# nyu-systems/Grendel-GS

Measured on AMD Instinct MI355X. Metric: training iters/sec (fwd+bwd), higher is better.
Workload: dtype f32

## Files before the change

grendel-gs_amd/csrc/api.hip:

```cpp
#include "common.h"

extern "C" {

const char *gsr_error_string(int code) {
    if (code == 0) return "success";
    if (code == GSR_EINVAL) return "gsraster: invalid argument";
    if (code == GSR_ENOSPACE) return "gsraster: workspace too small";
    if (code == GSR_ERETRY) return "gsraster: pair count valid, bounded sort must be repeated";
    if (code == GSR_EFAULT)
        return "gsraster: a persistent binning kernel of an earlier call timed out at a grid barrier (hung or preempted "
               "device); that view's lists are incomplete; the look-back pipeline is used from now on";
    if (code > 0) return hipGetErrorString((hipError_t)code);
    return "gsraster: unknown error";
}

int gsr_abi_version(void) { return 14; }

int gsr_get_block_xy(int *block_x, int *block_y, int *one_dim_block) {
    if (!block_x || !block_y || !one_dim_block) return GSR_EINVAL;
    *block_x = GSR_BLOCK_X;
    *block_y = GSR_BLOCK_Y;
    *one_dim_block = GSR_ONE_DIM_BLOCK;
    return 0;
}
// ... 189 lines not shown
                              const uint8_t *compute_locally, const float *bg, const float *final_T,
                              const int32_t *n_contrib, const float *dL_dpixels, float *dL_record,
                              const float *out_color, void *seg_ws, size_t seg_bytes, int row_lo, int row_hi,
                              int record_is_zero, double *acc64, uint8_t *touched, gsr_stream_t stream) {
    if (P < 0 || width <= 0 || height <= 0) return GSR_EINVAL;
    if (P == 0) return 0;
    if (!ranges || !compute_locally || !bg || !final_T || !n_contrib || !dL_dpixels || !means2D || !conic_opacity ||
        !rgb || !dL_record || !acc64)
        return GSR_EINVAL;
    return gsr_launch_composite_backward(P, width, height, ranges, point_list, means2D, conic_opacity, rgb,
                                         compute_locally, bg, final_T, n_contrib, dL_dpixels, dL_record, out_color,
                                         seg_ws, seg_bytes, row_lo, row_hi, record_is_zero ? 1 : 0,
                                         reinterpret_cast<hipStream_t>(stream), acc64, touched);
}

int gsr_render_backward(int P, int width, int height, const int32_t *ranges, const uint32_t *point_list,
                        const float *means2D, const float *conic_opacity, const float *rgb,
                        const uint8_t *compute_locally, const float *bg, const float *final_T,
                        const int32_t *n_contrib, const float *dL_dpixels, float *dL_record, gsr_stream_t stream) {
    if (P < 0 || width <= 0 || height <= 0) return GSR_EINVAL;
    if (P == 0) return 0;
    if (!ranges || !compute_locally || !bg || !final_T || !n_contrib || !dL_dpixels || !means2D || !conic_opacity ||
        !rgb || !dL_record)
        return GSR_EINVAL;
    return gsr_launch_composite_backward(P, width, height, ranges, point_list, means2D, conic_opacity, rgb,
                                         compute_locally, bg, final_T, n_contrib, dL_dpixels, dL_record, nullptr,
                                         nullptr, 0, 0, 0, 0, reinterpret_cast<hipStream_t>(stream));
}

}
// ... 1 lines not shown
```

grendel-gs_amd/csrc/common.h:

```cpp
#pragma once
#include <hip/hip_runtime.h>
#include <stdint.h>

#include "../../include/gsraster.h"

#define GSR_WAVE 64

#define GSR_LAUNCH_CHECK()                         \
    do {                                           \
        hipError_t e__ = hipGetLastError();        \
        if (e__ != hipSuccess) return (int)e__;    \
    } while (0)

#define GSR_HIP(expr)                              \
    do {                                           \
        hipError_t e__ = (expr);                   \
        if (e__ != hipSuccess) return (int)e__;    \
    } while (0)

static inline int gsr_div_up(long long a, long long b) { return (int)((a + b - 1) / b); }

__device__ __forceinline__ int gsr_xcd_span_of_block(int b, int nwg) {
#ifdef GSR_NO_XCD_MAP
    return b;
// ... 75 lines not shown
                                  hipStream_t stream);
int gsr_launch_preprocess_backward(int P, int D, int M, const float *means3D, const float *scales,
                                   float scale_modifier, const float *rotations, const float *shs,
                                   const float *shs_rest, const float *opacities_raw, const float *viewmatrix, const float *projmatrix, const float *campos, int W,
                                   int H, float tanfovx, float tanfovy, const int32_t *radii, const float *cov3D,
                                   const uint8_t *clamped, const float *dL_dmeans2D, const float *dL_dconic_opacity,
                                   const float *dL_drgb, int grad_row_stride, float *dL_dmeans3D, float *dL_dscales, float *dL_drotations,
                                   float *dL_dshs, float *dL_dshs_rest, float *dL_dopacities, hipStream_t stream);
int gsr_launch_local2j(int P, int W, int H, int ws, const float *means2D, const int32_t *radii, const int32_t *div,
                       uint8_t *out, hipStream_t stream);

int gsr_launch_composite_forward(int P, int W, int H, const int32_t *ranges, const uint32_t *point_list,
                                 const float *means2D, const float *conic_opacity, const float *rgb,
                                 const uint8_t *compute_locally, const float *bg, float *out_color, float *final_T,
                                 int32_t *n_contrib, void *seg_ws, size_t seg_bytes, int row_lo, int row_hi,
                                 void *zero_ptr, size_t zero_bytes, hipStream_t stream);
size_t gsr_composite_seg_bytes(int W, int H);
int gsr_launch_composite_backward(int P, int W, int H, const int32_t *ranges, const uint32_t *point_list,
                                  const float *means2D, const float *conic_opacity, const float *rgb,
                                  const uint8_t *compute_locally, const float *bg, const float *final_T,
                                  const int32_t *n_contrib, const float *dL_dpixels, float *dL_record,
                                  const float *out_color, void *seg_ws, size_t seg_bytes, int row_lo, int row_hi,
                                  int record_is_zero, hipStream_t stream, double *acc64 = nullptr,
                                  uint8_t *touched = nullptr);
```

grendel-gs_amd/csrc/composite.hip:

```cpp
#include "common.h"

namespace {

constexpr float LOG2E = 1.4426950408889634f;
constexpr float ALPHA_MIN = 1.0f / 255.0f;
constexpr float T_STOP = 0.0001f;

__device__ unsigned long long g_walked[2];

#ifdef GSR_STATS
__device__ unsigned long long g_stats[8];
#define GSR_STAT(i, v) do { const unsigned long long sv__ = (unsigned long long)(v); if (lane == 0) atomicAdd(&g_stats[i], sv__); } while (0)
#else
#define GSR_STAT(i, v) do { } while (0)
#endif

struct Entry {
    float x, y;
    float a2, b2, c2;
    float o;
    bool relevant;
};

#ifndef GSR_NO_LOG2O
// ... 125 lines not shown
    return 64 + sizeof(uint32_t) * (size_t)cap + sizeof(int32_t) * (size_t)tiles * SEG_MAXJ + sizeof(float) * 1024 * (size_t)cap;
}
inline SegWs seg_ws_of(void *ws, int tiles, uint32_t cap) {
    SegWs w{};
    if (!ws) return w;
    char *b = reinterpret_cast<char *>(ws);
    w.hdr = reinterpret_cast<uint32_t *>(b);
    w.queue = reinterpret_cast<uint32_t *>(b + 64);
    w.seg_slot = reinterpret_cast<int32_t *>(b + 64 + sizeof(uint32_t) * (size_t)cap);
    w.ckpt = reinterpret_cast<float *>(b + 64 + sizeof(uint32_t) * (size_t)cap + sizeof(int32_t) * (size_t)tiles * SEG_MAXJ);
    w.cap = cap;
    return w;
}
constexpr uint32_t SEG_CAP = 8192;

__device__ __forceinline__ void k8_checkpoint(const SegWs &seg, int *s_slot, int tile, int c, int lane,
                                                        int wave, float T, float c0, float c1, float c2) {
    const int j = c / SEG_LEN - 1;
    int slot = 0;
    if (lane == 0) {
        int v = atomicCAS(&s_slot[j], -1, -2);
        if (v == -1) {
            const uint32_t k = atomicAdd(seg.hdr, 1u);
            v = k < seg.cap ? (int)k : -3;
            if (v >= 0) {
                seg.queue[k] = (uint32_t)tile * 32u + (uint32_t)(j + 1);
                seg.seg_slot[(size_t)tile * SEG_MAXJ + j] = v;
            }
            __hip_atomic_store(&s_slot[j], v, __ATOMIC_RELEASE, __HIP_MEMORY_SCOPE_WORKGROUP);
        } else {
// ... 7 lines not shown
        ck[0] = T;
        ck[256] = c0;
        ck[512] = c1;
        ck[768] = c2;
    }
}

template <bool SEG, bool BAND>
__global__ void __launch_bounds__(256)
composite_forward_kernel(int W, int H, int gx, const int2 *__restrict__ ranges,
                         const uint32_t *__restrict__ point_list, const float2 *__restrict__ means2D,
                         const float4 *__restrict__ conic_opacity, const float *__restrict__ rgb,
                         const uint8_t *__restrict__ compute_locally, const float *__restrict__ bg,
                         float *__restrict__ out_color, float *__restrict__ final_T, int32_t *__restrict__ n_contrib,
                         const SegWs seg, int band_first, int band_tiles, uint4 *__restrict__ zero16,
                         size_t zero16_n) {
    const size_t HW = (size_t)H * W;
    for (size_t i = (size_t)blockIdx.x * 256 + threadIdx.x; i < zero16_n; i += (size_t)gridDim.x * 256)
        zero16[i] = make_uint4(0u, 0u, 0u, 0u);
    int tile;
    bool idle = false;
    if (BAND) {
        if (band_first < 0) {
            const int gy = (H + GSR_BLOCK_Y - 1) / GSR_BLOCK_Y;
            int2 hull = ranges[gx * gy];
            if (hull.x < 0 || hull.y > gy || hull.x >= hull.y) hull = make_int2(0, 0);
            band_first = hull.x * gx;
            band_tiles = min((hull.y - hull.x) * gx, band_tiles);
            idle = (int)blockIdx.x >= band_tiles;
        }
        tile = band_first + (idle ? 0 : gsr_xcd_span_of_block(blockIdx.x, band_tiles));
// ... 6 lines not shown
        const size_t p1 = (size_t)min(H, ((band_first + band_tiles) / gx) * GSR_BLOCK_Y) * W;
        const size_t nout = n0 + (HW - p1);
        for (size_t i = (size_t)blockIdx.x * 256 + threadIdx.x; i < nout; i += (size_t)gridDim.x * 256) {
            const size_t q = i < n0 ? i : p1 + (i - n0);
            out_color[q] = 0.f;
            out_color[HW + q] = 0.f;
            out_color[2 * HW + q] = 0.f;
            final_T[q] = 1.f;
            n_contrib[q] = 0;
        }
    };
    if (idle) {
        clear_outside();
        return;
    }
    const int lane = threadIdx.x & 63, wave = threadIdx.x >> 6;
    const int tx = tile % gx, ty = tile / gx;
    const int qx0 = tx * GSR_BLOCK_X + (wave & 1) * 8, qy0 = ty * GSR_BLOCK_Y + (wave >> 1) * 8;
    const int px = qx0 + (lane & 7), py = qy0 + (lane >> 3);
    const bool inside = px < W && py < H;
    const size_t pid = (size_t)py * W + px;

    if (!compute_locally[tile]) {
        if (inside) {
            out_color[pid] = 0.f;
            out_color[HW + pid] = 0.f;
            out_color[2 * HW + pid] = 0.f;
            final_T[pid] = 1.f;
            n_contrib[pid] = 0;
        }
        clear_outside();
// ... 30 lines not shown
        float r = 0.f, g = 0.f, b = 0.f;
        if (e.relevant) {
            r = rgb[3 * (size_t)id];
            g = rgb[3 * (size_t)id + 1];
            b = rgb[3 * (size_t)id + 2];
        }
        unsigned long long m = __ballot(e.relevant);
        GSR_STAT(0, __popcll(__ballot(have)));
        GSR_STAT(1, __popcll(m));
        const int nrel = __popcll(m);
        if (e.relevant) pair_store(wslab, __popcll(m & ((1ull << lane) - 1ull)), e, r, g, b);
        {
            const int pad = (-nrel) & 3, slot = nrel + lane / 9;
            if (lane < 9 * pad) wslab[(slot >> 1) * PREC + 2 * (lane % 9) + (slot & 1)] = 0.f;
        }
        for (int p0 = 0; p0 < nrel; p0 += 4) {
            float al[4];
            bool ok[4];
            int kk[4];
            v2f cr[2], cg[2], cb[2];
#pragma unroll
            for (int h = 0; h < 2; h++) {
                const PairRec pr = pair_load(wslab, (p0 >> 1) + h);
                const v2f pe = pair_exponent(pr, pxf, pyf);
                cr[h] = pr.r;
                cg[h] = pr.g;
                cb[h] = pr.b;
#pragma unroll
                for (int u = 0; u < 2; u++) {
                    const bool live = m != 0;
// ... 37 lines not shown
    if (inside) {
        out_color[pid] = C0 + T * bg[0];
        out_color[HW + pid] = C1 + T * bg[1];
        out_color[2 * HW + pid] = C2 + T * bg[2];
        final_T[pid] = T;
        n_contrib[pid] = last;
    }
    clear_outside();
}

typedef float f32x4 __attribute__((ext_vector_type(4)));

constexpr int MB = 8;
constexpr int MSTR = 66;

template <typename Acc>
__device__ __forceinline__ void
composite_backward_segment(const int tile, const int sidx, int W, int H, int gx, const int2 *__restrict__ ranges,
                           const uint32_t *__restrict__ point_list, const float2 *__restrict__ means2D,
                           const float4 *__restrict__ conic_opacity, const float *__restrict__ rgb,
                           const uint8_t *__restrict__ compute_locally, const float *__restrict__ bg,
                           const float *__restrict__ final_T, const int32_t *__restrict__ n_contrib,
                           const float *__restrict__ dL_dpixels, Acc *__restrict__ dL_record,
                           const float *__restrict__ out_color, const SegWs &seg, uint8_t *__restrict__ touched) {
    if (!compute_locally[tile]) return;
    const int lane = threadIdx.x & 63, wave = threadIdx.x >> 6;
    const int tx = tile % gx, ty = tile / gx;
    const int qx0 = tx * GSR_BLOCK_X + (wave & 1) * 8, qy0 = ty * GSR_BLOCK_Y + (wave >> 1) * 8;
    const int px = qx0 + (lane & 7), py = qy0 + (lane >> 3);
    const bool inside = px < W && py < H;
    const size_t pid = (size_t)py * W + px;
    const size_t HW = (size_t)H * W;
    const int2 range = ranges[tile];
    const float pxf = (float)px, pyf = (float)py;

    const int c_lo = sidx * SEG_LEN;
    int end_slot = -1;
    if (seg.seg_slot && sidx < SEG_MAXJ) end_slot = seg.seg_slot[(size_t)tile * SEG_MAXJ + sidx];
    const int c_hi = end_slot >= 0 ? c_lo + SEG_LEN : 0x7fffffff;
// ... 66 lines not shown

    float T = T_final;
    float rho = 0.f;
    if (end_slot >= 0 && last > c_hi) {
        const float *ck = seg.ckpt + (size_t)end_slot * 1024 + wave * 64 + lane;
        T = ck[0];
        const float r0 = out_color[pid] - T_final * bg[0] - ck[256];
        const float r1 = out_color[HW + pid] - T_final * bg[1] - ck[512];
        const float r2 = out_color[2 * HW + pid] - T_final * bg[2] - ck[768];
        rho = (r0 * g0 + r1 * g1 + r2 * g2) * __builtin_amdgcn_rcpf(T);
    }

    const int c0 = ((bmax - 1) / 64) * 64;
    uint32_t id_cur = (c0 + lane < wmax) ? point_list[range.x + c0 + lane] : 0u;
    uint32_t id_nxt = (c0 >= c_lo + 64 && c0 - 64 + lane < wmax) ? point_list[range.x + c0 - 64 + lane] : 0u;
    RawEntry raw = load_raw(c0 + lane < wmax, id_cur, means2D, conic_opacity, rgb);

    for (int c = c0; c >= c_lo; c -= 64) {
        float *acc_tab = sacc[wave];
        const bool have_nxt = c >= c_lo + 64 && c - 64 + lane < wmax;
        const RawEntry raw_nxt = load_raw(have_nxt, id_nxt, means2D, conic_opacity, rgb);
        const uint32_t id_nxt2 = (c >= c_lo + 128 && c - 128 + lane < wmax) ? point_list[range.x + c - 128 + lane] : 0u;
        if (c < wmax) {
            const bool have = c + lane < wmax;
            Entry e;
            e.x = raw.xy.x;
            e.y = raw.xy.y;
            e.a2 = -0.5f * LOG2E * raw.co.x;
            e.b2 = -LOG2E * raw.co.y;
            e.c2 = -0.5f * LOG2E * raw.co.z;
            e.o = entry_opacity_term(raw.co.w);
            e.relevant = have && gsr_can_touch_box(raw.xy, raw.co, (float)qx0, (float)qy0, (float)qx0 + 7.0f, (float)qy0 + 7.0f);
            unsigned long long m = __ballot(e.relevant);
            GSR_STAT(0, __popcll(__ballot(have)));
            GSR_STAT(1, __popcll(m));
            GSR_STAT(6, 1);
            if (e.relevant) pair_store(wslab, __popcll((m >> lane) >> 1), e, raw.r, raw.g, raw.b);
            if (wave == wbest) {
                float *fe = &fslab[7 * lane];
                fe[0] = e.x;  fe[1] = e.y;  fe[2] = e.a2;  fe[3] = e.b2;  fe[4] = e.c2;
                fe[5] = __uint_as_float(id_cur);
                fe[6] = raw.co.w;
            }
            unsigned long long sk = 0ull;
            auto contract_batch = [&](int filled) {
                __builtin_amdgcn_wave_barrier();
                f32x4 acc = {0.f, 0.f, 0.f, 0.f}, acc1 = {0.f, 0.f, 0.f, 0.f};
#pragma unroll
// ... 101 lines not shown
                if (val != 0.f) {
                    const uint32_t id = __float_as_uint(sout[10 * e + 9]);
                    atomicAdd(dL_record + 9 * (size_t)id + col, (Acc)val);
                    if (touched) touched[id] = 1;
                }
#else
                asm volatile("" ::"v"(val));
#endif
            }
        }
#pragma unroll
        for (int i = 0; i < 9; i++) acc_tab[64 * i + lane] = 0.f;
        raw = raw_nxt;
        id_cur = id_nxt;
        id_nxt = id_nxt2;
    }
}

template <typename Acc>
__global__ void __launch_bounds__(256, 4)
composite_backward_kernel(int W, int H, int gx, int tiles, const int2 *__restrict__ ranges,
                          const uint32_t *__restrict__ point_list, const float2 *__restrict__ means2D,
                          const float4 *__restrict__ conic_opacity, const float *__restrict__ rgb,
                          const uint8_t *__restrict__ compute_locally, const float *__restrict__ bg,
                          const float *__restrict__ final_T, const int32_t *__restrict__ n_contrib,
                          const float *__restrict__ dL_dpixels, Acc *__restrict__ dL_record,
                          const float *__restrict__ out_color, const SegWs seg, int band_first, int band_tiles,
                          uint8_t *__restrict__ touched) {
    const int nstatic = band_tiles > 0 ? band_tiles : tiles;
    const bool worker = (int)blockIdx.x >= nstatic;
    if (band_first < 0 && band_tiles > 0) {
        const int gy = tiles / gx;
        int2 hull = ranges[tiles];
        if (hull.x < 0 || hull.y > gy || hull.x >= hull.y) hull = make_int2(0, 0);
        band_first = hull.x * gx;
        band_tiles = min((hull.y - hull.x) * gx, band_tiles);
        if (!worker && (int)blockIdx.x >= band_tiles) return;
    }
    __shared__ uint32_t s_item;
    const uint32_t count = worker ? min(seg.hdr[0], seg.cap) : 0u;
    for (;;) {
        int tile, sidx = 0;
        if (worker) {
            __syncthreads();
            if (threadIdx.x == 0) s_item = atomicAdd(&seg.hdr[1], 1u);
            __syncthreads();
            const uint32_t t = s_item;
            if (t >= count) return;
            const uint32_t item = seg.queue[t];
            tile = (int)(item >> 5);
            sidx = (int)(item & 31u);
        } else {
            tile = band_tiles > 0 ? band_first + gsr_xcd_span_of_block(blockIdx.x, band_tiles)
                                  : composite_tile_of_block(ranges, gx, tiles);
        }
        composite_backward_segment(tile, sidx, W, H, gx, ranges, point_list, means2D, conic_opacity, rgb,
                                   compute_locally, bg, final_T, n_contrib, dL_dpixels, dL_record, out_color, seg, touched);
        if (!worker) return;
    }
}

}

extern "C" int gsr_composite_walked(unsigned long long *out2, int reset) {
    if (!out2) return GSR_EINVAL;
    GSR_HIP(hipMemcpyFromSymbol(out2, HIP_SYMBOL(g_walked), sizeof(unsigned long long) * 2));
    if (reset) {
        const unsigned long long z[2] = {0ull, 0ull};
        GSR_HIP(hipMemcpyToSymbol(HIP_SYMBOL(g_walked), z, sizeof(z)));
    }
    return 0;
}

#ifdef GSR_STATS
extern "C" int gsr_debug_stats(unsigned long long *out8, int reset) {
    if (hipMemcpyFromSymbol(out8, HIP_SYMBOL(g_stats), sizeof(unsigned long long) * 8) != hipSuccess) return -1;
    if (reset) {
        unsigned long long z[8] = {0, 0, 0, 0, 0, 0, 0, 0};
        if (hipMemcpyToSymbol(HIP_SYMBOL(g_stats), z, sizeof(z)) != hipSuccess) return -1;
    }
    return 0;
}
#endif

size_t gsr_composite_seg_bytes(int W, int H) {
    const int gx = (W + GSR_BLOCK_X - 1) / GSR_BLOCK_X, gy = (H + GSR_BLOCK_Y - 1) / GSR_BLOCK_Y;
    return seg_ws_bytes(gx * gy, SEG_CAP);
}

int gsr_launch_composite_forward(int P, int W, int H, const int32_t *ranges, const uint32_t *point_list,
                                 const float *means2D, const float *conic_opacity, const float *rgb,
                                 const uint8_t *compute_locally, const float *bg, float *out_color, float *final_T,
                                 int32_t *n_contrib, void *seg_ws, size_t seg_bytes, int row_lo, int row_hi,
                                 void *zero_ptr, size_t zero_bytes, hipStream_t stream) {
    (void)P;
    if (zero_bytes && (!zero_ptr || ((uintptr_t)zero_ptr & 15) || (zero_bytes & 3))) return GSR_EINVAL;
    const size_t zero16_n = zero_bytes / 16;
    if (zero_bytes & 15)
        GSR_HIP(hipMemsetAsync(reinterpret_cast<char *>(zero_ptr) + zero16_n * 16, 0, zero_bytes & 15, stream));
    const int gx = (W + GSR_BLOCK_X - 1) / GSR_BLOCK_X, gy = (H + GSR_BLOCK_Y - 1) / GSR_BLOCK_Y;
    const bool dyn = row_lo == -1 && row_hi > 0 && row_hi <= gy;
    const bool band = dyn || (row_lo >= 0 && row_lo < row_hi && row_hi <= gy && !(row_lo == 0 && row_hi == gy));
    const int band_first = dyn ? -1 : band ? row_lo * gx : 0;
    const int band_tiles = dyn ? row_hi * gx : band ? (row_hi - row_lo) * gx : 0;
    if (seg_ws && seg_bytes < seg_ws_bytes(gx * gy, SEG_CAP)) return GSR_ENOSPACE;
    const SegWs seg = seg_ws_of(seg_ws, gx * gy, SEG_CAP);
    if (seg_ws) GSR_HIP(hipMemsetAsync(seg_ws, 0, 64, stream));
    auto launch = [&](auto kern) {
        hipLaunchKernelGGL(kern, dim3(band ? band_tiles : gx * gy), dim3(256), 0, stream, W, H, gx,
                           reinterpret_cast<const int2 *>(ranges), point_list, reinterpret_cast<const float2 *>(means2D),
                           reinterpret_cast<const float4 *>(conic_opacity), rgb, compute_locally, bg, out_color, final_T,
                           n_contrib, seg, band_first, band_tiles, reinterpret_cast<uint4 *>(zero_ptr), zero16_n);
    };
    if (seg_ws && band) launch(composite_forward_kernel<true, true>);
    else if (seg_ws) launch(composite_forward_kernel<true, false>);
    else if (band) launch(composite_forward_kernel<false, true>);
    else launch(composite_forward_kernel<false, false>);
    GSR_LAUNCH_CHECK();
    return 0;
}

__global__ void record_from_f64_kernel(const double *__restrict__ acc, float *__restrict__ rec, size_t n) {
    const size_t i = (size_t)blockIdx.x * blockDim.x + threadIdx.x;
    if (i < n) rec[i] = (float)acc[i];
}

__global__ void record_from_f64_touched_kernel(const double *__restrict__ acc, float *__restrict__ rec,
// ... 2 lines not shown
    if (i >= P || !touched[i]) return;
    const double *a = acc + 9 * (size_t)i;
    float *r = rec + 9 * (size_t)i;
    double v[9];
#pragma unroll
    for (int k = 0; k < 9; k++) v[k] = a[k];
#pragma unroll
    for (int k = 0; k < 9; k++) r[k] = (float)v[k];
}

int gsr_launch_composite_backward(int P, int W, int H, const int32_t *ranges, const uint32_t *point_list,
                                  const float *means2D, const float *conic_opacity, const float *rgb,
                                  const uint8_t *compute_locally, const float *bg, const float *final_T,
                                  const int32_t *n_contrib, const float *dL_dpixels, float *dL_record,
                                  const float *out_color, void *seg_ws, size_t seg_bytes, int row_lo, int row_hi,
                                  int record_is_zero, hipStream_t stream, double *acc64, uint8_t *touched) {
    if (!record_is_zero || !acc64) touched = nullptr;
    if (!record_is_zero) {
        if (acc64) GSR_HIP(hipMemsetAsync(acc64, 0, sizeof(double) * 9 * (size_t)P, stream));
        else GSR_HIP(hipMemsetAsync(dL_record, 0, sizeof(float) * 9 * (size_t)P, stream));
    }
    if (P == 0) return 0;
    const int gx = (W + GSR_BLOCK_X - 1) / GSR_BLOCK_X, gy = (H + GSR_BLOCK_Y - 1) / GSR_BLOCK_Y;
    const bool dyn = row_lo == -1 && row_hi > 0 && row_hi <= gy;
    const bool band = dyn || (row_lo >= 0 && row_lo < row_hi && row_hi <= gy && !(row_lo == 0 && row_hi == gy));
    const int band_first = dyn ? -1 : band ? row_lo * gx : 0;
    const int band_tiles = dyn ? row_hi * gx : band ? (row_hi - row_lo) * gx : 0;
    if (seg_ws && (seg_bytes < seg_ws_bytes(gx * gy, SEG_CAP) || !out_color)) return GSR_EINVAL;
    const SegWs seg = seg_ws_of(seg_ws, gx * gy, SEG_CAP);
    if (seg_ws) GSR_HIP(hipMemsetAsync(reinterpret_cast<char *>(seg_ws) + sizeof(uint32_t), 0, sizeof(uint32_t), stream));
    const dim3 grid((band ? band_tiles : gx * gy) + (seg_ws ? SEG_WORKERS : 0));
    if (acc64) {
        hipLaunchKernelGGL(composite_backward_kernel<double>, grid, dim3(256), 0, stream, W, H, gx, gx * gy,
                           reinterpret_cast<const int2 *>(ranges), point_list, reinterpret_cast<const float2 *>(means2D),
                           reinterpret_cast<const float4 *>(conic_opacity), rgb, compute_locally, bg, final_T, n_contrib,
                           dL_dpixels, acc64, out_color, seg, band_first, band_tiles, touched);
        GSR_LAUNCH_CHECK();
        const size_t n = 9 * (size_t)P;
        if (touched)
            hipLaunchKernelGGL(record_from_f64_touched_kernel, dim3((unsigned)((P + 255) / 256)), dim3(256), 0, stream,
                               acc64, dL_record, touched, P);
        else
            hipLaunchKernelGGL(record_from_f64_kernel, dim3((unsigned)((n + 255) / 256)), dim3(256), 0, stream, acc64,
                               dL_record, n);
    } else {
        hipLaunchKernelGGL(composite_backward_kernel<float>, grid, dim3(256), 0, stream, W, H, gx, gx * gy,
                           reinterpret_cast<const int2 *>(ranges), point_list, reinterpret_cast<const float2 *>(means2D),
                           reinterpret_cast<const float4 *>(conic_opacity), rgb, compute_locally, bg, final_T, n_contrib,
                           dL_dpixels, dL_record, out_color, seg, band_first, band_tiles,
                           static_cast<uint8_t *>(nullptr));
    }
    GSR_LAUNCH_CHECK();
    return 0;
}
```

grendel-gs_amd/diff_gaussian_rasterization/__init__.py:

```python
import contextlib
import ctypes
import os
from typing import NamedTuple

import torch
import torch.nn as nn

from . import _lib
from ._lib import check, lib

__all__ = ["GaussianRasterizationSettings", "GaussianRasterizer", "_C", "load_image_tiles_by_pos",
           "merge_image_tiles_by_pos", "set_timing_mode", "fused_l1_ssim_band", "fused_band_loss", "fused_activations", "pack_camera",
           "preprocess_gaussians_raw_batched", "knn_mean_dist2", "group_rows", "gather_rows", "densify_plan", "densify_move", "exchange_need",
           "exchange_count", "exchange_pack", "exchange_pack_slab", "exchange_unpack", "zeros_async", "scatter_add_rows", "densify_stats",
           "set_tie_order", "scatter_rows", "local_pixels", "GraphCapture", "capturing"]

BLOCK_X, BLOCK_Y, ONE_DIM_BLOCK_SIZE = 16, 16, 256

_TIMING_MODE = "auto"
_last_backward_ms = 0.0


def set_timing_mode(mode):
    global _TIMING_MODE
# ... 651 lines not shown
        _SORT_SCRATCH[key] = buf
    return buf


def release_workspaces():
    _SORT_SCRATCH.clear()
    _MAX_PAIRS.clear()


_SPECULATIVE_SORT = [os.environ.get("GSR_SPECULATIVE_SORT", "1") != "0"]
_SEGMENTS = [{"0": False, "always": "always"}.get(os.environ.get("GSR_SEGMENTS", "1"), True)]
_BAND_GRID = [os.environ.get("GSR_BAND_GRID", "1") != "0"]
_ZERO_IN_FORWARD = [os.environ.get("GSR_ZERO_IN_FORWARD", "1") != "0"]
_KEEP_BACKWARD_BUFFERS = [None]
_TOUCHED_ROWS = [os.environ.get("GSR_TOUCHED_ROWS", "1") != "0"]


def set_list_segments(on):
    _SEGMENTS[0] = "always" if on == "always" else bool(on)


def set_speculative_sort(on):
    _SPECULATIVE_SORT[0] = bool(on)


GSR_ERETRY = -3


_PERSIST_USER = [None]
_LAST_SEGMENTS = [0]
# ... 261 lines not shown
            lists = [point_list]
            record = acc64 = touched = None
            zero_buf, zero_bytes = None, 0
            if any(ctx.needs_input_grad[:3]) and P > 0 and _ZERO_IN_FORWARD[0]:
                if _TOUCHED_ROWS[0]:
                    zero_bytes = 108 * P + ((P + 15) & ~15)
                    zero_buf = torch.empty((zero_bytes,), dtype=torch.uint8, device=dev)
                    acc64 = zero_buf[:72 * P].view(torch.float64).view(P, 9)
                    record = zero_buf[72 * P:108 * P].view(torch.float32).view(P, 9)
                    touched = zero_buf[108 * P:109 * P]
                else:
                    record = torch.empty((P, 9), dtype=torch.float32, device=dev)
                    zero_buf = acc64 = torch.empty((P, 9), dtype=torch.float64, device=dev)
                    zero_bytes = 72 * P
            ctx.record = (record, acc64, touched) if record is not None else None

            def launch_k8(meta_D):
                with kernel_timer.range("composite_forward", P=P, D=meta_D, **ctx.px_meta) as k8t, \
                        zhx_range(cuda_args, "70 render time"):
                    check(lib.gsr_render_forward_seg_z(P, W, H, _ptr(ranges), _ptr(lists[0]), _ptr(means2D),
                                                       _ptr(conic_opacity), _ptr(rgb), _ptr(mask), _ptr(bg), _ptr(out),
                                                       _ptr(final_T), _ptr(n_contrib), _ptr(seg_ws), seg_bytes, row_lo,
                                                       row_hi, _ptr(zero_buf), zero_bytes,
                                                       _stream()), "gsr_render_forward_seg_z")
                return k8t

            k8t = launch_k8(D)
            if _CAPTURE[0] is not None:
                _CAPTURE[0].stamp("fwd1", id(stats))
            ctx.seg = (seg_ws, seg_bytes, row_lo, row_hi)
            ctx.lists = lists
            ctx.num_rendered = D
            _RenderGaussians.last_num_rendered = D
            if pend is not None:
                def settle(ctx=ctx, pend=pend, kt=kt, k8t=k8t, lists=lists):
                    D, again = pend.finish()
                    kt.meta["D"] = k8t.meta["D"] = D
                    ctx.num_rendered = D
                    _RenderGaussians.last_num_rendered = D
                    if again is not None:
                        lists[0] = again
                        with _on(pend.dev), torch.cuda.stream(pend.stream):
                            launch_k8(D)
                    return D

                collector = cuda_args.get("_gsr_pending") if isinstance(cuda_args, dict) else None
# ... 36 lines not shown
        if _KEEP_BACKWARD_BUFFERS[0] is not None:
            _KEEP_BACKWARD_BUFFERS[0].append(pair)
        d_means2D, d_rgb, d_conic_opacity = record[:, 0:2], record[:, 2:5], record[:, 5:9]
        timing = ctx.timing
        with _on(dev):
            if timing != "off":
                ev0 = torch.cuda.Event(enable_timing=True)
                ev1 = torch.cuda.Event(enable_timing=True)
                ev0.record(current_stream(dev))
            cap_stats = ctx.cuda_args.get("stats_collector") if isinstance(ctx.cuda_args, dict) else None
            if _CAPTURE[0] is not None:
                _CAPTURE[0].stamp("bwd0", id(cap_stats))
            with kernel_timer.range("composite_backward", P=P, D=ctx.num_rendered, **ctx.px_meta), \
                    zhx_range(ctx.cuda_args, "b10 render time"):
                seg_ws, seg_bytes, row_lo, row_hi = ctx.seg
                check(lib.gsr_render_backward_seg_t(P, W, H, _ptr(ranges), _ptr(point_list), _ptr(means2D),
                                                    _ptr(conic_opacity), _ptr(rgb), _ptr(mask), _ptr(bg), _ptr(final_T),
                                                    _ptr(n_contrib), _ptr(g_out), _ptr(record), _ptr(out_img),
                                                    _ptr(seg_ws), seg_bytes, row_lo, row_hi, 1 if record_is_zero else 0,
                                                    _ptr(acc64), _ptr(touched), _stream()), "gsr_render_backward_seg_t")
            if _CAPTURE[0] is not None:
                _CAPTURE[0].stamp("bwd1", id(cap_stats))
            if timing != "off":
                ev1.record(current_stream(dev))
        stats = ctx.cuda_args.get("stats_collector") if isinstance(ctx.cuda_args, dict) else None
        if stats is not None and timing != "off":
            f0, f1 = ctx.fwd_events
            if timing == "sync":
                ev1.synchronize()
                _last_backward_ms = float(ev0.elapsed_time(ev1))
                stats["forward_render_time"] = float(f0.elapsed_time(f1))
                stats["backward_render_time"] = _last_backward_ms
            else:
                if timing == "deferred":
                    stats["_fwd_events"] = (f0, f1)
# ... 554 lines not shown
```

grendel-gs_amd/diff_gaussian_rasterization/_lib.py:

```python
import ctypes
import os

_HERE = os.path.dirname(os.path.abspath(__file__))
LIB_PATH = os.environ.get("GSRASTER_LIB") or os.path.join(_HERE, "libgsraster.so")

c_int, c_float, c_void_p, c_size_t, c_int64 = (ctypes.c_int, ctypes.c_float, ctypes.c_void_p, ctypes.c_size_t,
                                                ctypes.c_int64)

SIGNATURES = {
    "gsr_error_string": (ctypes.c_char_p, [c_int]),
    "gsr_abi_version": (c_int, []),
    "gsr_get_block_xy": (c_int, [ctypes.POINTER(c_int)] * 3),
    "gsr_preprocess_forward": (c_int, [c_int, c_int, c_int, c_void_p, c_void_p, c_float, c_void_p, c_void_p, c_void_p,
                                       c_void_p, c_void_p, c_void_p, c_int, c_int, c_float, c_float, c_void_p,
                                       c_void_p, c_void_p, c_void_p, c_void_p, c_void_p, c_void_p, c_void_p]),
    "gsr_preprocess_backward": (c_int, [c_int, c_int, c_int, c_void_p, c_void_p, c_float, c_void_p, c_void_p,
                                        c_void_p, c_void_p, c_void_p, c_int, c_int, c_float, c_float] +
                                [c_void_p] * 6 + [c_int] + [c_void_p] * 6),
    "gsr_get_local2j_ids_bool": (c_int, [c_int, c_int, c_int, c_int, c_void_p, c_void_p, c_void_p, c_void_p,
                                         c_void_p]),
    "gsr_bin_prepare_bytes": (c_size_t, [c_int, c_int, c_int]),
    "gsr_bin_prepare": (c_int, [c_int, c_int, c_int, c_void_p, c_void_p, c_void_p, c_void_p, c_void_p, c_void_p,
                                c_size_t, ctypes.POINTER(c_int64), c_void_p]),
    "gsr_bin_sort_bytes": (c_size_t, [c_int, c_int64, c_int, c_int]),
# ... 80 lines not shown
    "gsr_flag_if_greater": (c_int, [c_void_p, ctypes.c_uint32, c_void_p, ctypes.c_uint32, c_void_p, c_void_p]),
    "gsr_render_seg_bytes": (c_size_t, [c_int, c_int]),
    "gsr_render_forward_seg": (c_int, [c_int, c_int, c_int, c_void_p, c_void_p, c_void_p, c_void_p, c_void_p, c_void_p,
                                       c_void_p, c_void_p, c_void_p, c_void_p, c_void_p, c_size_t, c_int, c_int,
                                       c_void_p]),
    "gsr_render_backward_seg": (c_int, [c_int, c_int, c_int] + [c_void_p] * 13 + [c_size_t, c_int, c_int, c_void_p]),
    "gsr_render_forward_seg_z": (c_int, [c_int, c_int, c_int, c_void_p, c_void_p, c_void_p, c_void_p, c_void_p,
                                         c_void_p, c_void_p, c_void_p, c_void_p, c_void_p, c_void_p, c_size_t, c_int,
                                         c_int, c_void_p, c_size_t, c_void_p]),
    "gsr_render_backward_seg_z": (c_int, [c_int, c_int, c_int] + [c_void_p] * 13 + [c_size_t, c_int, c_int, c_int,
                                                                                   c_void_p]),
    "gsr_render_backward_seg_d": (c_int, [c_int, c_int, c_int] + [c_void_p] * 13 + [c_size_t, c_int, c_int, c_int,
                                                                                   c_void_p, c_void_p]),
    "gsr_render_backward_seg_t": (c_int, [c_int, c_int, c_int] + [c_void_p] * 13 + [c_size_t, c_int, c_int, c_int,
                                                                                   c_void_p, c_void_p, c_void_p]),
    "gsr_composite_walked": (c_int, [ctypes.POINTER(ctypes.c_ulonglong), c_int]),
    "gsr_publish_flag": (c_int, [c_void_p, c_void_p, c_void_p, ctypes.c_uint32, c_void_p]),
    "gsr_exchange_check": (c_int, [c_void_p, c_void_p, c_int, c_int, c_int, ctypes.c_uint64, c_int, c_void_p,
                                   ctypes.c_uint32, ctypes.c_uint32, c_void_p, c_void_p]),
    "gsr_activate_forward": (c_int, [c_int, c_int] + [c_void_p] * 10),
    "gsr_activate_backward": (c_int, [c_int, c_int] + [c_void_p] * 13),
    "gsr_render_backward": (c_int, [c_int, c_int, c_int] + [c_void_p] * 12),
}

ABI_VERSION = 14


def _load():
    if not os.path.exists(LIB_PATH):
        raise ImportError(
# ... 22 lines not shown
```

include/gsraster.h:

```cpp
#ifndef GSRASTER_H
#define GSRASTER_H

#include <stddef.h>
#include <stdint.h>

#ifdef __cplusplus
extern "C" {
#endif

#define GSR_BLOCK_X 16
#define GSR_BLOCK_Y 16
#define GSR_ONE_DIM_BLOCK 256

#define GSR_EINVAL (-1)
#define GSR_ENOSPACE (-2)
#define GSR_ERETRY (-3)
#define GSR_EFAULT (-4)

typedef void *gsr_stream_t;

const char *gsr_error_string(int code);

int gsr_abi_version(void);

// ... 94 lines not shown
                              const int32_t *n_contrib, const float *dL_dpixels, float *dL_record, const float *out_color,
                              void *seg_ws, size_t seg_bytes, int row_lo, int row_hi, int record_is_zero,
                              gsr_stream_t stream);
int gsr_render_backward_seg_d(int P, int width, int height, const int32_t *ranges, const uint32_t *point_list,
                              const float *means2D, const float *conic_opacity, const float *rgb,
                              const uint8_t *compute_locally, const float *bg, const float *final_T,
                              const int32_t *n_contrib, const float *dL_dpixels, float *dL_record, const float *out_color,
                              void *seg_ws, size_t seg_bytes, int row_lo, int row_hi, int record_is_zero,
                              double *acc64, gsr_stream_t stream);
int gsr_render_backward_seg_t(int P, int width, int height, const int32_t *ranges, const uint32_t *point_list,
                              const float *means2D, const float *conic_opacity, const float *rgb,
                              const uint8_t *compute_locally, const float *bg, const float *final_T,
                              const int32_t *n_contrib, const float *dL_dpixels, float *dL_record, const float *out_color,
                              void *seg_ws, size_t seg_bytes, int row_lo, int row_hi, int record_is_zero,
                              double *acc64, uint8_t *touched, gsr_stream_t stream);
int gsr_composite_walked(unsigned long long *out2, int reset);

int gsr_l1_ssim_num_partials(int channels, int rows, int width);
int gsr_l1_ssim_forward(int channels, int rows, int width, const float *image, int64_t image_channel_stride,
                        const uint8_t *gt, float *partials, float *dm_dmu1, float *dm_dE11, float *dm_dE12,
                        gsr_stream_t stream);
int gsr_l1_ssim_backward(int channels, int rows, int width, const float *image, int64_t image_channel_stride,
                         const uint8_t *gt, const float *dm_dmu1, const float *dm_dE11, const float *dm_dE12,
                         const float *grad_l1_sum, const float *grad_ssim_sum, float scale_l1, float scale_ssim,
                         float *grad_image, int64_t grad_channel_stride, gsr_stream_t stream);
int gsr_l1_ssim_forward_band(int channels, int rows_capacity, int width, const float *image, int64_t image_channel_stride,
                             const uint8_t *gt, float *partials, float *dm_dmu1, float *dm_dE11, float *dm_dE12,
                             const int32_t *band_rows, gsr_stream_t stream);
int gsr_l1_ssim_backward_band(int channels, int rows_capacity, int width, const float *image,
                              int64_t image_channel_stride, const uint8_t *gt, const float *dm_dmu1, const float *dm_dE11,
// ... 142 lines not shown
```

Measured before the change: 816.3.

## Cache per-wave relevance ballots from forward composite for reuse in backward

The forward composite kernel now writes each wave's 64-bit relevance ballot per 64-entry chunk into a mask buffer. The backward kernel reads these masks instead of recomputing gsr_can_touch_box for every entry, with the mask loads prefetched two chunks ahead alongside the point IDs. The aim is to remove redundant quadric-edge culling arithmetic in the backward pass. The cost is an extra global write in the forward pass, an extra buffer of up to a size budget, and a dependence on forward and backward computing identical chunk and wave layouts.

```diff
diff --git a/grendel-gs_amd/csrc/api.hip b/grendel-gs_amd/csrc/api.hip
--- a/grendel-gs_amd/csrc/api.hip
+++ b/grendel-gs_amd/csrc/api.hip
@@ -227,6 +227,49 @@
                                          reinterpret_cast<hipStream_t>(stream), acc64, touched);
 }
 
+size_t gsr_render_mask_bytes(size_t capacity, int width, int height) {
+    if (width <= 0 || height <= 0) return 0;
+    return gsr_composite_mask_bytes(capacity, width, height);
+}
+
+size_t gsr_render_mask_slot(int list_start, int tile, int chunk) {
+    if (list_start < 0 || tile < 0 || chunk < 0) return (size_t)-1;
+    return gsr_composite_mask_slot(list_start, tile, chunk);
+}
+
+int gsr_render_forward_seg_m(int P, int width, int height, const int32_t *ranges, const uint32_t *point_list,
+                             const float *means2D, const float *conic_opacity, const float *rgb,
+                             const uint8_t *compute_locally, const float *bg, float *out_color, float *final_T,
+                             int32_t *n_contrib, void *seg_ws, size_t seg_bytes, int row_lo, int row_hi, void *zero_ptr,
+                             size_t zero_bytes, void *mask_ptr, size_t mask_slots, gsr_stream_t stream) {
+    if (P < 0 || width <= 0 || height <= 0) return GSR_EINVAL;
+    if (!ranges || !compute_locally || !bg || !out_color || !final_T || !n_contrib) return GSR_EINVAL;
+    if (P > 0 && (!means2D || !conic_opacity || !rgb)) return GSR_EINVAL;
+    return gsr_launch_composite_forward(P, width, height, ranges, point_list, means2D, conic_opacity, rgb,
+                                        compute_locally, bg, out_color, final_T, n_contrib, seg_ws, seg_bytes, row_lo,
+                                        row_hi, zero_ptr, zero_bytes, reinterpret_cast<hipStream_t>(stream), mask_ptr,
+                                        mask_ptr ? mask_slots : 0);
+}
+
+int gsr_render_backward_seg_m(int P, int width, int height, const int32_t *ranges, const uint32_t *point_list,
+                              const float *means2D, const float *conic_opacity, const float *rgb,
+                              const uint8_t *compute_locally, const float *bg, const float *final_T,
+                              const int32_t *n_contrib, const float *dL_dpixels, float *dL_record,
+                              const float *out_color, void *seg_ws, size_t seg_bytes, int row_lo, int row_hi,
+                              int record_is_zero, double *acc64, uint8_t *touched, const void *mask_ptr,
+                              size_t mask_slots, gsr_stream_t stream) {
+    if (P < 0 || width <= 0 || height <= 0) return GSR_EINVAL;
+    if (P == 0) return 0;
+    if (!ranges || !compute_locally || !bg || !final_T || !n_contrib || !dL_dpixels || !means2D || !conic_opacity ||
+        !rgb || !dL_record || !acc64)
+        return GSR_EINVAL;
+    return gsr_launch_composite_backward(P, width, height, ranges, point_list, means2D, conic_opacity, rgb,
+                                         compute_locally, bg, final_T, n_contrib, dL_dpixels, dL_record, out_color,
+                                         seg_ws, seg_bytes, row_lo, row_hi, record_is_zero ? 1 : 0,
+                                         reinterpret_cast<hipStream_t>(stream), acc64, touched, mask_ptr,
+                                         mask_ptr ? mask_slots : 0);
+}
+
 int gsr_render_backward(int P, int width, int height, const int32_t *ranges, const uint32_t *point_list,
                         const float *means2D, const float *conic_opacity, const float *rgb,
                         const uint8_t *compute_locally, const float *bg, const float *final_T,
diff --git a/grendel-gs_amd/csrc/common.h b/grendel-gs_amd/csrc/common.h
--- a/grendel-gs_amd/csrc/common.h
+++ b/grendel-gs_amd/csrc/common.h
@@ -113,12 +113,15 @@
                                  const float *means2D, const float *conic_opacity, const float *rgb,
                                  const uint8_t *compute_locally, const float *bg, float *out_color, float *final_T,
                                  int32_t *n_contrib, void *seg_ws, size_t seg_bytes, int row_lo, int row_hi,
-                                 void *zero_ptr, size_t zero_bytes, hipStream_t stream);
+                                 void *zero_ptr, size_t zero_bytes, hipStream_t stream, void *cull = nullptr,
+                                 size_t cull_slots = 0);
 size_t gsr_composite_seg_bytes(int W, int H);
+size_t gsr_composite_mask_bytes(size_t capacity, int W, int H);
+size_t gsr_composite_mask_slot(int list_start, int tile, int chunk);
 int gsr_launch_composite_backward(int P, int W, int H, const int32_t *ranges, const uint32_t *point_list,
                                   const float *means2D, const float *conic_opacity, const float *rgb,
                                   const uint8_t *compute_locally, const float *bg, const float *final_T,
                                   const int32_t *n_contrib, const float *dL_dpixels, float *dL_record,
                                   const float *out_color, void *seg_ws, size_t seg_bytes, int row_lo, int row_hi,
                                   int record_is_zero, hipStream_t stream, double *acc64 = nullptr,
-                                  uint8_t *touched = nullptr);
+                                  uint8_t *touched = nullptr, const void *cull = nullptr, size_t cull_slots = 0);
diff --git a/grendel-gs_amd/csrc/composite.hip b/grendel-gs_amd/csrc/composite.hip
--- a/grendel-gs_amd/csrc/composite.hip
+++ b/grendel-gs_amd/csrc/composite.hip
@@ -163,6 +163,11 @@
 }
 constexpr uint32_t SEG_CAP = 8192;
 
+__host__ __device__ inline size_t cull_mask_slots(size_t capacity, int tiles) { return (capacity >> 6) + (size_t)tiles + 1; }
+__host__ __device__ inline uint32_t cull_mask_slot(int list_start, int tile, int chunk) {
+    return (uint32_t)(list_start >> 6) + (uint32_t)tile + (uint32_t)chunk;
+}
+
 __device__ __forceinline__ void k8_checkpoint(const SegWs &seg, int *s_slot, int tile, int c, int lane,
                                                         int wave, float T, float c0, float c1, float c2) {
     const int j = c / SEG_LEN - 1;
@@ -200,7 +205,7 @@
                          const uint8_t *__restrict__ compute_locally, const float *__restrict__ bg,
                          float *__restrict__ out_color, float *__restrict__ final_T, int32_t *__restrict__ n_contrib,
                          const SegWs seg, int band_first, int band_tiles, uint4 *__restrict__ zero16,
-                         size_t zero16_n) {
+                         size_t zero16_n, unsigned long long *__restrict__ cull, uint32_t cull_slots) {
     const size_t HW = (size_t)H * W;
     for (size_t i = (size_t)blockIdx.x * 256 + threadIdx.x; i < zero16_n; i += (size_t)gridDim.x * 256)
         zero16[i] = make_uint4(0u, 0u, 0u, 0u);
@@ -237,7 +242,7 @@
         clear_outside();
         return;
     }
-    const int lane = threadIdx.x & 63, wave = threadIdx.x >> 6;
+    const int lane = threadIdx.x & 63, wave = __builtin_amdgcn_readfirstlane(threadIdx.x >> 6);
     const int tx = tile % gx, ty = tile / gx;
     const int qx0 = tx * GSR_BLOCK_X + (wave & 1) * 8, qy0 = ty * GSR_BLOCK_Y + (wave >> 1) * 8;
     const int px = qx0 + (lane & 7), py = qy0 + (lane >> 3);
@@ -298,6 +303,10 @@
             const int pad = (-nrel) & 3, slot = nrel + lane / 9;
             if (lane < 9 * pad) wslab[(slot >> 1) * PREC + 2 * (lane % 9) + (slot & 1)] = 0.f;
         }
+        if (cull) {
+            const uint32_t slot = cull_mask_slot(range.x, tile, c >> 6);
+            if (lane == 0 && slot < cull_slots) cull[4 * (size_t)slot + wave] = m;
+        }
         for (int p0 = 0; p0 < nrel; p0 += 4) {
             float al[4];
             bool ok[4];
@@ -365,7 +374,7 @@
 constexpr int MB = 8;
 constexpr int MSTR = 66;
 
-template <typename Acc>
+template <typename Acc, bool CULL>
 __device__ __forceinline__ void
 composite_backward_segment(const int tile, const int sidx, int W, int H, int gx, const int2 *__restrict__ ranges,
                            const uint32_t *__restrict__ point_list, const float2 *__restrict__ means2D,
@@ -373,7 +382,8 @@
                            const uint8_t *__restrict__ compute_locally, const float *__restrict__ bg,
                            const float *__restrict__ final_T, const int32_t *__restrict__ n_contrib,
                            const float *__restrict__ dL_dpixels, Acc *__restrict__ dL_record,
-                           const float *__restrict__ out_color, const SegWs &seg, uint8_t *__restrict__ touched) {
+                           const float *__restrict__ out_color, const SegWs &seg, uint8_t *__restrict__ touched,
+                           const unsigned long long *__restrict__ cull, uint32_t cull_slots) {
     if (!compute_locally[tile]) return;
     const int lane = threadIdx.x & 63, wave = threadIdx.x >> 6;
     const int tx = tile % gx, ty = tile / gx;
@@ -470,13 +480,26 @@
     const int c0 = ((bmax - 1) / 64) * 64;
     uint32_t id_cur = (c0 + lane < wmax) ? point_list[range.x + c0 + lane] : 0u;
     uint32_t id_nxt = (c0 >= c_lo + 64 && c0 - 64 + lane < wmax) ? point_list[range.x + c0 - 64 + lane] : 0u;
-    RawEntry raw = load_raw(c0 + lane < wmax, id_cur, means2D, conic_opacity, rgb);
+    RawEntry raw;
+    const uint32_t cull_wave = __builtin_amdgcn_readfirstlane(wave);
+    auto cull_word = [&](int c) -> unsigned long long {
+        const uint32_t slot = __builtin_amdgcn_readfirstlane(min(cull_mask_slot(range.x, tile, c >> 6), cull_slots - 1u));
+        return cull[4 * (size_t)slot + cull_wave];
+    };
+    unsigned long long mk_cur = 0ull, mk_nxt = 0ull;
+    if (CULL) {
+        mk_cur = cull_word(c0);
+        if (c0 >= c_lo + 64) mk_nxt = cull_word(c0 - 64);
+    }
+    raw = load_raw(c0 + lane < wmax, id_cur, means2D, conic_opacity, rgb);
 
     for (int c = c0; c >= c_lo; c -= 64) {
         float *acc_tab = sacc[wave];
         const bool have_nxt = c >= c_lo + 64 && c - 64 + lane < wmax;
         const RawEntry raw_nxt = load_raw(have_nxt, id_nxt, means2D, conic_opacity, rgb);
         const uint32_t id_nxt2 = (c >= c_lo + 128 && c - 128 + lane < wmax) ? point_list[range.x + c - 128 + lane] : 0u;
+        unsigned long long mk_nxt2 = 0ull;
+        if (CULL && c >= c_lo + 128) mk_nxt2 = cull_word(c - 128);
         if (c < wmax) {
             const bool have = c + lane < wmax;
             Entry e;
@@ -486,8 +509,17 @@
             e.b2 = -LOG2E * raw.co.y;
             e.c2 = -0.5f * LOG2E * raw.co.z;
             e.o = entry_opacity_term(raw.co.w);
-            e.relevant = have && gsr_can_touch_box(raw.xy, raw.co, (float)qx0, (float)qy0, (float)qx0 + 7.0f, (float)qy0 + 7.0f);
-            unsigned long long m = __ballot(e.relevant);
+            unsigned long long m;
+            if (CULL) {
+                const int nh = __builtin_amdgcn_readfirstlane(wmax - c);
+                const uint32_t lo = __builtin_amdgcn_readfirstlane((uint32_t)mk_cur);
+                const uint32_t hi = __builtin_amdgcn_readfirstlane((uint32_t)(mk_cur >> 32));
+                m = (((unsigned long long)hi << 32) | lo) & (nh >= 64 ? ~0ull : (1ull << nh) - 1ull);
+                e.relevant = (lane < 32 ? (uint32_t)m >> lane : (uint32_t)(m >> 32) >> (lane - 32)) & 1u;
+            } else {
+                e.relevant = have && gsr_can_touch_box(raw.xy, raw.co, (float)qx0, (float)qy0, (float)qx0 + 7.0f, (float)qy0 + 7.0f);
+                m = __ballot(e.relevant);
+            }
             GSR_STAT(0, __popcll(__ballot(have)));
             GSR_STAT(1, __popcll(m));
             GSR_STAT(6, 1);
@@ -619,10 +651,12 @@
         raw = raw_nxt;
         id_cur = id_nxt;
         id_nxt = id_nxt2;
-    }
-}
-
-template <typename Acc>
+        mk_cur = mk_nxt;
+        mk_nxt = mk_nxt2;
+    }
+}
+
+template <typename Acc, bool CULL>
 __global__ void __launch_bounds__(256, 4)
 composite_backward_kernel(int W, int H, int gx, int tiles, const int2 *__restrict__ ranges,
                           const uint32_t *__restrict__ point_list, const float2 *__restrict__ means2D,
@@ -631,7 +665,8 @@
                           const float *__restrict__ final_T, const int32_t *__restrict__ n_contrib,
                           const float *__restrict__ dL_dpixels, Acc *__restrict__ dL_record,
                           const float *__restrict__ out_color, const SegWs seg, int band_first, int band_tiles,
-                          uint8_t *__restrict__ touched) {
+                          uint8_t *__restrict__ touched, const unsigned long long *__restrict__ cull,
+                          uint32_t cull_slots) {
     const int nstatic = band_tiles > 0 ? band_tiles : tiles;
     const bool worker = (int)blockIdx.x >= nstatic;
     if (band_first < 0 && band_tiles > 0) {
@@ -659,8 +694,9 @@
             tile = band_tiles > 0 ? band_first + gsr_xcd_span_of_block(blockIdx.x, band_tiles)
                                   : composite_tile_of_block(ranges, gx, tiles);
         }
-        composite_backward_segment(tile, sidx, W, H, gx, ranges, point_list, means2D, conic_opacity, rgb,
-                                   compute_locally, bg, final_T, n_contrib, dL_dpixels, dL_record, out_color, seg, touched);
+        composite_backward_segment<Acc, CULL>(tile, sidx, W, H, gx, ranges, point_list, means2D, conic_opacity, rgb,
+                                              compute_locally, bg, final_T, n_contrib, dL_dpixels, dL_record, out_color,
+                                              seg, touched, cull, cull_slots);
         if (!worker) return;
     }
 }
@@ -688,6 +724,13 @@
 }
 #endif
 
+size_t gsr_composite_mask_bytes(size_t capacity, int W, int H) {
+    const int gx = (W + GSR_BLOCK_X - 1) / GSR_BLOCK_X, gy = (H + GSR_BLOCK_Y - 1) / GSR_BLOCK_Y;
+    return 4 * sizeof(unsigned long long) * cull_mask_slots(capacity, gx * gy);
+}
+
+size_t gsr_composite_mask_slot(int list_start, int tile, int chunk) { return cull_mask_slot(list_start, tile, chunk); }
+
 size_t gsr_composite_seg_bytes(int W, int H) {
     const int gx = (W + GSR_BLOCK_X - 1) / GSR_BLOCK_X, gy = (H + GSR_BLOCK_Y - 1) / GSR_BLOCK_Y;
     return seg_ws_bytes(gx * gy, SEG_CAP);
@@ -697,8 +740,9 @@
                                  const float *means2D, const float *conic_opacity, const float *rgb,
                                  const uint8_t *compute_locally, const float *bg, float *out_color, float *final_T,
                                  int32_t *n_contrib, void *seg_ws, size_t seg_bytes, int row_lo, int row_hi,
-                                 void *zero_ptr, size_t zero_bytes, hipStream_t stream) {
+                                 void *zero_ptr, size_t zero_bytes, hipStream_t stream, void *cull, size_t cull_slots) {
     (void)P;
+    if (cull && (((uintptr_t)cull & 7) || cull_slots == 0 || cull_slots > 0xffffffffull)) return GSR_EINVAL;
     if (zero_bytes && (!zero_ptr || ((uintptr_t)zero_ptr & 15) || (zero_bytes & 3))) return GSR_EINVAL;
     const size_t zero16_n = zero_bytes / 16;
     if (zero_bytes & 15)
@@ -715,7 +759,8 @@
         hipLaunchKernelGGL(kern, dim3(band ? band_tiles : gx * gy), dim3(256), 0, stream, W, H, gx,
                            reinterpret_cast<const int2 *>(ranges), point_list, reinterpret_cast<const float2 *>(means2D),
                            reinterpret_cast<const float4 *>(conic_opacity), rgb, compute_locally, bg, out_color, final_T,
-                           n_contrib, seg, band_first, band_tiles, reinterpret_cast<uint4 *>(zero_ptr), zero16_n);
+                           n_contrib, seg, band_first, band_tiles, reinterpret_cast<uint4 *>(zero_ptr), zero16_n,
+                           reinterpret_cast<unsigned long long *>(cull), (uint32_t)cull_slots);
     };
     if (seg_ws && band) launch(composite_forward_kernel<true, true>);
     else if (seg_ws) launch(composite_forward_kernel<true, false>);
@@ -748,13 +793,16 @@
                                   const uint8_t *compute_locally, const float *bg, const float *final_T,
                                   const int32_t *n_contrib, const float *dL_dpixels, float *dL_record,
                                   const float *out_color, void *seg_ws, size_t seg_bytes, int row_lo, int row_hi,
-                                  int record_is_zero, hipStream_t stream, double *acc64, uint8_t *touched) {
+                                  int record_is_zero, hipStream_t stream, double *acc64, uint8_t *touched,
+                                  const void *cull, size_t cull_slots) {
     if (!record_is_zero || !acc64) touched = nullptr;
     if (!record_is_zero) {
         if (acc64) GSR_HIP(hipMemsetAsync(acc64, 0, sizeof(double) * 9 * (size_t)P, stream));
         else GSR_HIP(hipMemsetAsync(dL_record, 0, sizeof(float) * 9 * (size_t)P, stream));
     }
     if (P == 0) return 0;
+    if (cull && (((uintptr_t)cull & 7) || cull_slots == 0 || cull_slots > 0xffffffffull)) return GSR_EINVAL;
+    const unsigned long long *cw = reinterpret_cast<const unsigned long long *>(cull);
     const int gx = (W + GSR_BLOCK_X - 1) / GSR_BLOCK_X, gy = (H + GSR_BLOCK_Y - 1) / GSR_BLOCK_Y;
     const bool dyn = row_lo == -1 && row_hi > 0 && row_hi <= gy;
     const bool band = dyn || (row_lo >= 0 && row_lo < row_hi && row_hi <= gy && !(row_lo == 0 && row_hi == gy));
@@ -764,11 +812,15 @@
     const SegWs seg = seg_ws_of(seg_ws, gx * gy, SEG_CAP);
     if (seg_ws) GSR_HIP(hipMemsetAsync(reinterpret_cast<char *>(seg_ws) + sizeof(uint32_t), 0, sizeof(uint32_t), stream));
     const dim3 grid((band ? band_tiles : gx * gy) + (seg_ws ? SEG_WORKERS : 0));
+    auto launch = [&](auto kern, auto *sums, uint8_t *flags) {
+        hipLaunchKernelGGL(kern, grid, dim3(256), 0, stream, W, H, gx, gx * gy, reinterpret_cast<const int2 *>(ranges),
+                           point_list, reinterpret_cast<const float2 *>(means2D),
+                           reinterpret_cast<const float4 *>(conic_opacity), rgb, compute_locally, bg, final_T, n_contrib,
+                           dL_dpixels, sums, out_color, seg, band_first, band_tiles, flags, cw, (uint32_t)cull_slots);
+    };
     if (acc64) {
-        hipLaunchKernelGGL(composite_backward_kernel<double>, grid, dim3(256), 0, stream, W, H, gx, gx * gy,
-                           reinterpret_cast<const int2 *>(ranges), point_list, reinterpret_cast<const float2 *>(means2D),
-                           reinterpret_cast<const float4 *>(conic_opacity), rgb, compute_locally, bg, final_T, n_contrib,
-                           dL_dpixels, acc64, out_color, seg, band_first, band_tiles, touched);
+        if (cw) launch(composite_backward_kernel<double, true>, acc64, touched);
+        else launch(composite_backward_kernel<double, false>, acc64, touched);
         GSR_LAUNCH_CHECK();
         const size_t n = 9 * (size_t)P;
         if (touched)
@@ -778,11 +830,8 @@
             hipLaunchKernelGGL(record_from_f64_kernel, dim3((unsigned)((n + 255) / 256)), dim3(256), 0, stream, acc64,
                                dL_record, n);
     } else {
-        hipLaunchKernelGGL(composite_backward_kernel<float>, grid, dim3(256), 0, stream, W, H, gx, gx * gy,
-                           reinterpret_cast<const int2 *>(ranges), point_list, reinterpret_cast<const float2 *>(means2D),
-                           reinterpret_cast<const float4 *>(conic_opacity), rgb, compute_locally, bg, final_T, n_contrib,
-                           dL_dpixels, dL_record, out_color, seg, band_first, band_tiles,
-                           static_cast<uint8_t *>(nullptr));
+        if (cw) launch(composite_backward_kernel<float, true>, dL_record, static_cast<uint8_t *>(nullptr));
+        else launch(composite_backward_kernel<float, false>, dL_record, static_cast<uint8_t *>(nullptr));
     }
     GSR_LAUNCH_CHECK();
     return 0;
diff --git a/grendel-gs_amd/diff_gaussian_rasterization/__init__.py b/grendel-gs_amd/diff_gaussian_rasterization/__init__.py
--- a/grendel-gs_amd/diff_gaussian_rasterization/__init__.py
+++ b/grendel-gs_amd/diff_gaussian_rasterization/__init__.py
@@ -689,6 +689,9 @@
 _ZERO_IN_FORWARD = [os.environ.get("GSR_ZERO_IN_FORWARD", "1") != "0"]
 _KEEP_BACKWARD_BUFFERS = [None]
 _TOUCHED_ROWS = [os.environ.get("GSR_TOUCHED_ROWS", "1") != "0"]
+_CULL_MASKS = [os.environ.get("GSR_CULL_MASKS", "1") != "0"]
+CULL_MASK_BUDGET = 64 << 20
+_CULL_MASK_BUDGET = [int(os.environ.get("GSR_CULL_MASK_BUDGET", CULL_MASK_BUDGET))]
 
 
 def set_list_segments(on):
@@ -980,15 +983,30 @@
                     zero_buf = acc64 = torch.empty((P, 9), dtype=torch.float64, device=dev)
                     zero_bytes = 72 * P
             ctx.record = (record, acc64, touched) if record is not None else None
+            cull = [None, 0]
+            want_cull = any(ctx.needs_input_grad[:3]) and P > 0 and _CULL_MASKS[0]
+
+            def size_cull():
+                if not want_cull:
+                    return
+                nbytes = int(lib.gsr_render_mask_bytes(lists[0].numel(), W, H))
+                if nbytes > _CULL_MASK_BUDGET[0]:
+                    cull[0], cull[1] = None, 0
+                    return
+                if cull[0] is None or cull[0].numel() < nbytes:
+                    cull[0] = None
+                    cull[0] = torch.empty((nbytes,), dtype=torch.uint8, device=dev)
+                cull[1] = nbytes // 32
 
             def launch_k8(meta_D):
+                size_cull()
                 with kernel_timer.range("composite_forward", P=P, D=meta_D, **ctx.px_meta) as k8t, \
                         zhx_range(cuda_args, "70 render time"):
-                    check(lib.gsr_render_forward_seg_z(P, W, H, _ptr(ranges), _ptr(lists[0]), _ptr(means2D),
+                    check(lib.gsr_render_forward_seg_m(P, W, H, _ptr(ranges), _ptr(lists[0]), _ptr(means2D),
                                                        _ptr(conic_opacity), _ptr(rgb), _ptr(mask), _ptr(bg), _ptr(out),
                                                        _ptr(final_T), _ptr(n_contrib), _ptr(seg_ws), seg_bytes, row_lo,
-                                                       row_hi, _ptr(zero_buf), zero_bytes,
-                                                       _stream()), "gsr_render_forward_seg_z")
+                                                       row_hi, _ptr(zero_buf), zero_bytes, _ptr(cull[0]), cull[1],
+                                                       _stream()), "gsr_render_forward_seg_m")
                 return k8t
 
             k8t = launch_k8(D)
@@ -996,6 +1014,7 @@
                 _CAPTURE[0].stamp("fwd1", id(stats))
             ctx.seg = (seg_ws, seg_bytes, row_lo, row_hi)
             ctx.lists = lists
+            ctx.cull = cull
             ctx.num_rendered = D
             _RenderGaussians.last_num_rendered = D
             if pend is not None:
@@ -1062,11 +1081,13 @@
             with kernel_timer.range("composite_backward", P=P, D=ctx.num_rendered, **ctx.px_meta), \
                     zhx_range(ctx.cuda_args, "b10 render time"):
                 seg_ws, seg_bytes, row_lo, row_hi = ctx.seg
-                check(lib.gsr_render_backward_seg_t(P, W, H, _ptr(ranges), _ptr(point_list), _ptr(means2D),
+                cull_buf, cull_slots = ctx.cull
+                check(lib.gsr_render_backward_seg_m(P, W, H, _ptr(ranges), _ptr(point_list), _ptr(means2D),
                                                     _ptr(conic_opacity), _ptr(rgb), _ptr(mask), _ptr(bg), _ptr(final_T),
                                                     _ptr(n_contrib), _ptr(g_out), _ptr(record), _ptr(out_img),
                                                     _ptr(seg_ws), seg_bytes, row_lo, row_hi, 1 if record_is_zero else 0,
-                                                    _ptr(acc64), _ptr(touched), _stream()), "gsr_render_backward_seg_t")
+                                                    _ptr(acc64), _ptr(touched), _ptr(cull_buf), cull_slots, _stream()),
+                      "gsr_render_backward_seg_m")
             if _CAPTURE[0] is not None:
                 _CAPTURE[0].stamp("bwd1", id(cap_stats))
             if timing != "off":
diff --git a/grendel-gs_amd/diff_gaussian_rasterization/_lib.py b/grendel-gs_amd/diff_gaussian_rasterization/_lib.py
--- a/grendel-gs_amd/diff_gaussian_rasterization/_lib.py
+++ b/grendel-gs_amd/diff_gaussian_rasterization/_lib.py
@@ -118,6 +118,14 @@
                                                                                    c_void_p, c_void_p]),
     "gsr_render_backward_seg_t": (c_int, [c_int, c_int, c_int] + [c_void_p] * 13 + [c_size_t, c_int, c_int, c_int,
                                                                                    c_void_p, c_void_p, c_void_p]),
+    "gsr_render_mask_bytes": (c_size_t, [c_size_t, c_int, c_int]),
+    "gsr_render_mask_slot": (c_size_t, [c_int, c_int, c_int]),
+    "gsr_render_forward_seg_m": (c_int, [c_int, c_int, c_int, c_void_p, c_void_p, c_void_p, c_void_p, c_void_p,
+                                         c_void_p, c_void_p, c_void_p, c_void_p, c_void_p, c_void_p, c_size_t, c_int,
+                                         c_int, c_void_p, c_size_t, c_void_p, c_size_t, c_void_p]),
+    "gsr_render_backward_seg_m": (c_int, [c_int, c_int, c_int] + [c_void_p] * 13 + [c_size_t, c_int, c_int, c_int,
+                                                                                   c_void_p, c_void_p, c_void_p,
+                                                                                   c_size_t, c_void_p]),
     "gsr_composite_walked": (c_int, [ctypes.POINTER(ctypes.c_ulonglong), c_int]),
     "gsr_publish_flag": (c_int, [c_void_p, c_void_p, c_void_p, ctypes.c_uint32, c_void_p]),
     "gsr_exchange_check": (c_int, [c_void_p, c_void_p, c_int, c_int, c_int, ctypes.c_uint64, c_int, c_void_p,
diff --git a/include/gsraster.h b/include/gsraster.h
--- a/include/gsraster.h
+++ b/include/gsraster.h
@@ -132,6 +132,20 @@
                               const int32_t *n_contrib, const float *dL_dpixels, float *dL_record, const float *out_color,
                               void *seg_ws, size_t seg_bytes, int row_lo, int row_hi, int record_is_zero,
                               double *acc64, uint8_t *touched, gsr_stream_t stream);
+size_t gsr_render_mask_bytes(size_t capacity, int width, int height);
+size_t gsr_render_mask_slot(int list_start, int tile, int chunk);
+int gsr_render_forward_seg_m(int P, int width, int height, const int32_t *ranges, const uint32_t *point_list,
+                             const float *means2D, const float *conic_opacity, const float *rgb,
+                             const uint8_t *compute_locally, const float *bg, float *out_color, float *final_T,
+                             int32_t *n_contrib, void *seg_ws, size_t seg_bytes, int row_lo, int row_hi, void *zero_ptr,
+                             size_t zero_bytes, void *mask_ptr, size_t mask_slots, gsr_stream_t stream);
+int gsr_render_backward_seg_m(int P, int width, int height, const int32_t *ranges, const uint32_t *point_list,
+                              const float *means2D, const float *conic_opacity, const float *rgb,
+                              const uint8_t *compute_locally, const float *bg, const float *final_T,
+                              const int32_t *n_contrib, const float *dL_dpixels, float *dL_record, const float *out_color,
+                              void *seg_ws, size_t seg_bytes, int row_lo, int row_hi, int record_is_zero,
+                              double *acc64, uint8_t *touched, const void *mask_ptr, size_t mask_slots,
+                              gsr_stream_t stream);
 int gsr_composite_walked(unsigned long long *out2, int reset);
 
 int gsr_l1_ssim_num_partials(int channels, int rows, int width);
```

Result: no change. 809.2 (median of 2 runs) (-0.9%).
